# yunjinli/TRASE

Hardware: AMD Instinct MI355X
Metric: views/sec (fwd+bwd), 1080p, 300k Gaussians, 32-d feat (higher is better)
Workload: dtype f32 (channel contractions: 3-product bf16-split MFMA, fp32 accumulate)

## Files before the change

### include/trase_rast.h

```cpp
#ifndef TRASE_RAST_H
#define TRASE_RAST_H

#include <stddef.h>
#include <stdint.h>

#ifdef __cplusplus
extern "C" {
#endif

typedef void* trase_stream_t;

enum {
  TRASE_OK = 0,
  TRASE_ERR_INVALID = -1,
  TRASE_ERR_UNSUPPORTED = -2,
  TRASE_ERR_WORKSPACE = -3,
  TRASE_ERR_HIP = -4
};

typedef struct TraseRastSettings {
  int32_t image_height;
  int32_t image_width;
  float tanfovx;
  float tanfovy;
// ... 294 lines not shown
                               float* dL_dC_F, int32_t device, trase_stream_t stream);

int trase_nnfm_sizes(int32_t C, int32_t N1, int32_t N2, size_t* ws_bytes);
int trase_nnfm_forward(const float* feat1, const float* feats2, int32_t C, int32_t N1, int32_t N2, float* loss, void* ws,
                       size_t ws_bytes, int32_t device, trase_stream_t stream);
int trase_nnfm_backward(const float* feat1, const float* feats2, int32_t C, int32_t N1, int32_t N2, const float* g_loss,
                        const void* ws, size_t ws_bytes, float* dL_dfeat1, int32_t device, trase_stream_t stream);

int trase_adam_step(int32_t count, float* const* params, const float* const* grads, float* const* exp_avg,
                    float* const* exp_avg_sq, const int64_t* numel, const float* lr, const int64_t* step, double beta1,
                    double beta2, float eps, int32_t device, trase_stream_t stream);
int trase_adam_step_guarded(int32_t count, float* const* params, const float* const* grads, float* const* exp_avg,
                            float* const* exp_avg_sq, const int64_t* numel, const float* lr, const int64_t* step, double beta1,
                            double beta2, float eps, const void* guard, int32_t device, trase_stream_t stream);

int trase_prof_enable(int enable);
int trase_prof_report(char* buf, size_t buf_bytes);

int trase_selftest(int32_t device, trase_stream_t stream, char* msg, size_t msg_bytes);

int trase_selftest_sort(const uint32_t* keys, const uint32_t* vals, uint32_t n, uint32_t cap, int32_t bit_lo, int32_t bit_hi,
                        int32_t digit_bits, int32_t hist_copies, int32_t start, uint32_t flag_key, int32_t use_flag,
                        uint32_t sentinel, uint32_t* keys_out, uint32_t* vals_out, uint32_t* result, int32_t device,
                        trase_stream_t stream);
int trase_selftest_tile_ranges(const uint32_t* keys, uint32_t n, uint32_t cap, int32_t T, int32_t clear, uint32_t* ranges,
                               uint32_t* dbg, int32_t device, trase_stream_t stream);
int trase_selftest_zero_bytes(void* p, size_t bytes, int32_t device, trase_stream_t stream);

int trase_selftest_compact_live(const uint32_t* tiles, const uint32_t* keys, int32_t P, uint32_t* keys_out, uint32_t* ids_out,
                                uint32_t* live_ids_out, uint32_t* hdr_out, int32_t device, trase_stream_t stream);
int trase_selftest_scan_tiles(const uint32_t* tiles, const uint32_t* ids, const int32_t* radii, const float* xy, int32_t P,
                              uint32_t n_live, uint32_t cap, int32_t pack_bits, int32_t gx, int32_t gy, uint32_t overflow_in,
                              uint32_t* offsets_out, uint32_t* block_sums_out, uint32_t* hdr_out, int32_t device,
                              trase_stream_t stream);

const char* trase_last_error(void);
const char* trase_version(void);

int trase_densify_stats(const float* viewspace_grad, const int32_t* radii, float* xyz_gradient_accum, float* denom,
                        float* max_radii2D, int32_t P, int32_t device, trase_stream_t stream);
int trase_densify_stats_guarded(const float* viewspace_grad, const int32_t* radii, float* xyz_gradient_accum, float* denom,
                                float* max_radii2D, int32_t P, const void* guard, int32_t device, trase_stream_t stream);
int trase_densify_sizes(int32_t P, size_t* ws_bytes);
int trase_densify_plan(const float* xyz_gradient_accum, const float* denom, const float* scaling, const float* opacity,
                       int32_t P, float grad_threshold, float dense_extent, float min_opacity, int32_t use_screen_size,
                       float big_extent, int32_t* counts, void* ws, size_t ws_bytes, int32_t device,
                       trase_stream_t stream);
// ... 212 lines not shown
```

### trase_amd/_lib.py

```python
from __future__ import annotations

import ctypes as C
import os

import torch

_HERE = os.path.dirname(os.path.abspath(__file__))
LIB_PATH = os.environ.get("TRASE_RAST_LIB") or os.path.join(_HERE, "lib", "libtrase_rast.so")

c_float_p = C.POINTER(C.c_float)
FRAME_PLANAR = 1
LAYERS_MAX = 10
RIGID_STATE_FLOATS = 16


class RastSettings(C.Structure):
    _fields_ = [
        ("image_height", C.c_int32), ("image_width", C.c_int32),
        ("tanfovx", C.c_float), ("tanfovy", C.c_float),
        ("bg", C.c_void_p), ("scale_modifier", C.c_float),
        ("viewmatrix", C.c_void_p), ("projmatrix", C.c_void_p),
        ("sh_degree", C.c_int32), ("campos", C.c_void_p),
        ("prefiltered", C.c_int32), ("debug", C.c_int32),
        ("device", C.c_int32), ("variant", C.c_int32),
# ... 330 lines not shown
    ("trase_compose_sizes", C.c_int, [C.POINTER(C.c_int32), C.c_int32, C.c_int32, C.POINTER(C.c_int64)]),
    ("trase_compose_part", C.c_int, [C.POINTER(ComposePart), C.c_int64, C.c_int64, C.c_void_p, C.c_void_p, C.c_void_p, C.c_void_p,
                                     C.c_void_p, C.c_void_p, C.c_int32, C.c_void_p]),
    ("trase_evaluate_frame", C.c_int, [C.POINTER(EvalFrame), C.POINTER(RastWorkspace), C.c_int32, C.c_void_p]),
    ("trase_layers_pack", C.c_int, [C.POINTER(C.c_void_p), C.c_int32, C.c_int32, C.c_void_p, C.c_int32, C.c_void_p]),
    ("trase_layers_finish", C.c_int, [C.c_void_p, C.POINTER(RastWorkspace), C.c_void_p, C.c_int32, C.c_int32, C.c_int32, C.c_void_p,
                                      C.c_void_p, C.c_void_p, C.c_int32, C.c_void_p]),
    ("trase_fps_sample", C.c_int, [C.c_void_p, C.c_int32, C.c_void_p, C.c_int32, C.c_void_p, C.c_int32, C.c_void_p, C.c_void_p,
                                   C.c_void_p, C.c_int32, C.c_void_p]),
    ("trase_trajectory_append", C.c_int, [C.c_void_p, C.c_int32, C.c_void_p, C.c_int32, C.c_void_p, C.c_int32, C.c_void_p]),
    ("trase_trajectory_draw", C.c_int, [C.c_void_p, C.c_int32, C.c_int32, C.c_int32, C.c_int32, C.POINTER(C.c_double * 16),
                                        C.c_int32, C.c_int32, C.c_void_p, C.c_void_p, C.c_void_p, C.c_int32, C.c_void_p]),
    ("trase_present_frame", C.c_int, [C.c_void_p, C.c_int32, C.c_int32, C.c_int32, C.c_int32, C.c_int32, C.c_void_p, C.c_void_p,
                                      C.c_void_p, C.c_float, C.c_void_p, C.c_void_p, C.c_int32, C.c_void_p]),
    ("trase_adam_step", C.c_int, [C.c_int32, C.c_void_p, C.c_void_p, C.c_void_p, C.c_void_p, C.c_void_p, C.c_void_p,
                                  C.c_void_p, C.c_double, C.c_double, C.c_float, C.c_int32, C.c_void_p]),
    ("trase_adam_step_guarded", C.c_int, [C.c_int32, C.c_void_p, C.c_void_p, C.c_void_p, C.c_void_p, C.c_void_p, C.c_void_p,
                                          C.c_void_p, C.c_double, C.c_double, C.c_float, C.c_void_p, C.c_int32, C.c_void_p]),
    ("trase_prof_enable", C.c_int, [C.c_int]),
    ("trase_prof_report", C.c_int, [C.c_char_p, C.c_size_t]),
    ("trase_selftest", C.c_int, [C.c_int32, C.c_void_p, C.c_char_p, C.c_size_t]),
    ("trase_selftest_sort", C.c_int, [C.c_void_p, C.c_void_p, C.c_uint32, C.c_uint32, C.c_int32, C.c_int32, C.c_int32, C.c_int32,
                                      C.c_int32, C.c_uint32, C.c_int32, C.c_uint32, C.c_void_p, C.c_void_p,
                                      C.POINTER(C.c_uint32 * 3), C.c_int32, C.c_void_p]),
    ("trase_selftest_tile_ranges", C.c_int, [C.c_void_p, C.c_uint32, C.c_uint32, C.c_int32, C.c_int32, C.c_void_p,
                                             C.POINTER(C.c_uint32 * 3), C.c_int32, C.c_void_p]),
    ("trase_selftest_zero_bytes", C.c_int, [C.c_void_p, C.c_size_t, C.c_int32, C.c_void_p]),
    ("trase_selftest_compact_live", C.c_int, [C.c_void_p, C.c_void_p, C.c_int32, C.c_void_p, C.c_void_p, C.c_void_p,
                                              C.POINTER(C.c_uint32 * 5), C.c_int32, C.c_void_p]),
    ("trase_selftest_scan_tiles", C.c_int, [C.c_void_p, C.c_void_p, C.c_void_p, C.c_void_p, C.c_int32, C.c_uint32, C.c_uint32,
                                            C.c_int32, C.c_int32, C.c_int32, C.c_uint32, C.c_void_p, C.c_void_p,
                                            C.POINTER(C.c_uint32 * 5), C.c_int32, C.c_void_p]),
    ("trase_last_error", C.c_char_p, []),
    ("trase_version", C.c_char_p, []),
]

_lib = None


def load() -> C.CDLL:
    global _lib
    if _lib is not None:
        return _lib
    if not os.path.exists(LIB_PATH):
        raise RuntimeError(
            f"trase_amd: HIP library not built: {LIB_PATH} is missing. Run "
            "`python -c 'import __graft_entry__ as g; g.build()'` (or `make -C trase_amd/csrc`). "
# ... 27 lines not shown
```

### trase_amd/csrc/binning.hip

```cpp
#include <stdlib.h>

#include "common.h"

namespace trase {

constexpr int RS_WAVES = RS_THREADS / WAVE;
constexpr int RS_SEG = WAVE * RS_ITEMS;

__device__ __forceinline__ uint32_t dev_n(const uint32_t* n_ptr, uint32_t cap) {
  const uint32_t n = *n_ptr;
  return n < cap ? n : cap;
}

__device__ __forceinline__ uint32_t rs_tile(uint32_t b, uint32_t nb_live) {
#ifdef TRASE_RS_NO_XCD_MAP
  return b;
#else
  return (uint32_t)xcd_block((int)b, (int)nb_live);
#endif
}

template <int DB, bool SMALL = false>
__global__ __launch_bounds__(RS_THREADS) void radix_hist_kernel(const uint32_t* __restrict__ keys,
                                                                const uint32_t* __restrict__ n_ptr, uint32_t cap,
                                                                int shift, uint32_t mask, uint32_t* __restrict__ hist,
                                                                uint32_t* __restrict__ digit_total, int nb_max,
                                                                uint32_t flag_key = 0u, uint32_t* __restrict__ flag_word = nullptr,
                                                                uint32_t* __restrict__ zero_from = nullptr, uint32_t zero_words = 0u) {
  constexpr int ND = 1 << DB;
  for (uint32_t i = blockIdx.x * RS_THREADS + threadIdx.x; i < zero_words; i += gridDim.x * RS_THREADS) zero_from[i] = 0u;
  const uint32_t n = dev_n(n_ptr, cap);
  const uint32_t nb_live = (n + RS_TILE - 1) / RS_TILE;
  if (blockIdx.x >= nb_live) return;
  const uint32_t tile = SMALL ? blockIdx.x : rs_tile(blockIdx.x, nb_live);
  const uint32_t base = tile * RS_TILE;
  __shared__ uint32_t h[ND];
#pragma unroll
  for (int d = threadIdx.x; d < ND; d += RS_THREADS) h[d] = 0;
  __syncthreads();
  const unsigned lane = threadIdx.x & 63;
  uint32_t kk[RS_ITEMS];
#pragma unroll
  for (int i = 0; i < RS_ITEMS; ++i) {
    const uint32_t idx = base + i * RS_THREADS + threadIdx.x;
    kk[i] = idx < n ? keys[idx] : 0u;
  }
#pragma unroll
  for (int i = 0; i < RS_ITEMS; ++i) {
    const uint32_t idx = base + i * RS_THREADS + threadIdx.x;
    const bool valid = idx < n;
    if (flag_word && valid && kk[i] == flag_key) atomicOr(flag_word, 2u);
    const uint32_t dg = valid ? ((kk[i] >> shift) & mask) : 0xffffffffu;
    const uint32_t prev = (uint32_t)__shfl_up((int)dg, 1);
    const bool start = valid && (lane == 0 || prev != dg);
    const unsigned long long starts = __ballot(start);
    const unsigned long long vmask = __ballot(valid);
    if (start) {
      const unsigned long long later = (lane == 63) ? 0ull : (starts >> (lane + 1));
      const unsigned nvalid = (unsigned)__popcll(vmask);
      const unsigned next = later ? (lane + 1 + (unsigned)__builtin_ctzll(later)) : nvalid;
      atomicAdd(&h[dg], next - lane);
    }
  }
  __syncthreads();
#pragma unroll
  for (int d = threadIdx.x; d < ND; d += RS_THREADS) hist[(size_t)d * nb_max + tile] = h[d];
}

__device__ __forceinline__ uint32_t block256_incl_scan(uint32_t v, uint32_t* part ) {
  const int lane = threadIdx.x & 63, wave = threadIdx.x >> 6;
  uint32_t x = v;
#pragma unroll
  for (int o = 1; o < 64; o <<= 1) {
    const uint32_t y = (uint32_t)__shfl_up((int)x, o);
    if (lane >= o) x += y;
  }
  if (lane == 63) part[wave] = x;
  __syncthreads();
  uint32_t add = 0;
#pragma unroll
  for (int w = 0; w < 3; ++w) add += (w < wave) ? part[w] : 0u;
  __syncthreads();
  return x + add;
}

__global__ __launch_bounds__(256) void radix_scan_kernel(const uint32_t* __restrict__ n_ptr, uint32_t cap,
                                                         uint32_t* __restrict__ hist,
                                                         uint32_t* __restrict__ digit_total, int nb_max) {
  const uint32_t n = dev_n(n_ptr, cap);
// ... 13 lines not shown
#pragma unroll
    for (int u = 0; u < 32; ++u) v[u] = (b_lo + u < b_hi) ? row[b_lo + u] : 0u;
#pragma unroll
    for (int u = 0; u < 32; ++u) mine += v[u];
    incl = block256_incl_scan(mine, sh);
    run = incl - mine;
#pragma unroll
    for (int u = 0; u < 32; ++u) {
      if (b_lo + u < b_hi) row[b_lo + u] = run;
      run += v[u];
    }
  } else {
    for (int b = b_lo; b < b_hi; ++b) mine += row[b];
    incl = block256_incl_scan(mine, sh);
    run = incl - mine;
    for (int b = b_lo; b < b_hi; ++b) { const uint32_t v = row[b]; row[b] = run; run += v; }
  }
  if (threadIdx.x == 255) carry = incl;
  __syncthreads();
  if (threadIdx.x == 0) digit_total[d] = carry;
}

template <bool IOTA, int DB, bool SMALL = false>
__global__ __launch_bounds__(RS_THREADS) void radix_scatter_kernel(
    const uint32_t* __restrict__ keys_in, const uint32_t* __restrict__ vals_in, uint32_t* __restrict__ keys_out,
    uint32_t* __restrict__ vals_out, const uint32_t* __restrict__ n_ptr, uint32_t cap, int shift, uint32_t mask,
    const uint32_t* __restrict__ hist, const uint32_t* __restrict__ digit_total, int nb_max,
    uint32_t* __restrict__ hist_next = nullptr, int shift_next = 0, uint32_t mask_next = 0u) {
  constexpr int ND = 1 << DB;
  constexpr int DPT = ND / RS_THREADS;
  const uint32_t n = dev_n(n_ptr, cap);
  const uint32_t nb_live = (n + RS_TILE - 1) / RS_TILE;
  if (blockIdx.x >= nb_live) return;
  const uint32_t tile = SMALL ? blockIdx.x : rs_tile(blockIdx.x, nb_live);
  const uint32_t base = tile * RS_TILE;
  __shared__ uint32_t wcount[RS_WAVES][ND];
  const int wave = threadIdx.x >> 6;
  const unsigned lane = threadIdx.x & 63;
#pragma unroll
  for (int w = 0; w < RS_WAVES; ++w)
#pragma unroll
    for (int d = threadIdx.x; d < ND; d += RS_THREADS) wcount[w][d] = 0;
  __syncthreads();
  uint32_t k[RS_ITEMS], v[RS_ITEMS], rk[RS_ITEMS];
  const unsigned long long lt = lanemask_lt();
  volatile uint32_t* cnt = wcount[wave];
  uint32_t my_digit_total[DPT], my_hist[DPT];
  if constexpr (SMALL) {
    const int nb = (int)((n + RS_TILE - 1) / RS_TILE);
#pragma unroll
    for (int j = 0; j < DPT; ++j) {
      const uint32_t* row = hist + (size_t)(threadIdx.x * DPT + j) * nb_max;
      uint32_t before = 0, total = 0;
      for (int b0 = 0; b0 < nb; b0 += 8) {
        uint32_t v8[8];
#pragma unroll
        for (int u = 0; u < 8; ++u) v8[u] = (b0 + u < nb) ? row[b0 + u] : 0u;
#pragma unroll
        for (int u = 0; u < 8; ++u) { total += v8[u]; before += (b0 + u < (int)tile) ? v8[u] : 0u; }
      }
      my_digit_total[j] = total; my_hist[j] = before;
    }
  } else {
#pragma unroll
  for (int j = 0; j < DPT; ++j) {
    my_digit_total[j] = digit_total[threadIdx.x * DPT + j];
    my_hist[j] = hist[(size_t)(threadIdx.x * DPT + j) * nb_max + tile];
  }
  }
#pragma unroll
  for (int i = 0; i < RS_ITEMS; ++i) {
    const uint32_t idx = base + wave * RS_SEG + i * WAVE + lane;
    const bool valid = idx < n;
    k[i] = valid ? keys_in[idx] : 0xffffffffu;
    v[i] = valid ? (IOTA ? idx : vals_in[idx]) : 0u;
  }
#pragma unroll
  for (int i = 0; i < RS_ITEMS; ++i) {
    const uint32_t idx = base + wave * RS_SEG + i * WAVE + lane;
    const bool valid = idx < n;
    const uint32_t dg = (k[i] >> shift) & mask;
    unsigned long long peers = __ballot(valid);
    const uint32_t dg0 = __builtin_amdgcn_readfirstlane(dg);
    if (!__all(!valid || dg == dg0)) {
#pragma unroll
      for (int bit = 0; bit < DB; ++bit) {
        const bool set = (dg >> bit) & 1u;
        const unsigned long long bal = __ballot(set);
        peers &= set ? bal : ~bal;
      }
    }
    const uint32_t in_round = (uint32_t)__popcll(peers & lt);
    const uint32_t total = (uint32_t)__popcll(peers);
    uint32_t old = 0;
    if (valid) {
      old = cnt[dg];
      if (in_round == 0) cnt[dg] = old + total;
    }
    rk[i] = old + in_round;
    __builtin_amdgcn_wave_barrier();
  }
  __syncthreads();
  __shared__ uint32_t gbase[ND], lstart[ND];
  __shared__ uint32_t st_k[RS_TILE], st_v[RS_TILE];
  __shared__ uint32_t part_a[4], part_b[4];
  {
    uint32_t cnt_d[DPT], sum_l = 0, sum_g = 0;
#pragma unroll
    for (int j = 0; j < DPT; ++j) {
      const int d = threadIdx.x * DPT + j;
      uint32_t tot = 0;
#pragma unroll
      for (int w = 0; w < RS_WAVES; ++w) {
        const uint32_t c = wcount[w][d];
        wcount[w][d] = tot;
        tot += c;
      }
      cnt_d[j] = tot;
      sum_l += tot;
      sum_g += my_digit_total[j];
    }
    uint32_t run_l = block256_incl_scan(sum_l, part_a) - sum_l;
    uint32_t run_g = block256_incl_scan(sum_g, part_b) - sum_g;
#pragma unroll
    for (int j = 0; j < DPT; ++j) {
      const int d = threadIdx.x * DPT + j;
      lstart[d] = run_l;
      gbase[d] = run_g + my_hist[j];
      run_l += cnt_d[j];
      run_g += my_digit_total[j];
    }
  }
  __syncthreads();
#pragma unroll
  for (int i = 0; i < RS_ITEMS; ++i) {
    const uint32_t idx = base + wave * RS_SEG + i * WAVE + lane;
    if (idx < n) {
      const uint32_t dg = (k[i] >> shift) & mask;
      const uint32_t lp = lstart[dg] + wcount[wave][dg] + rk[i];
      st_k[lp] = k[i];
      st_v[lp] = v[i];
    }
  }
  __syncthreads();
  const uint32_t nblk = min((uint32_t)RS_TILE, n - base);
  for (uint32_t j = threadIdx.x; j < nblk; j += RS_THREADS) {
    const uint32_t kk = st_k[j];
    const uint32_t dg = (kk >> shift) & mask;
    const uint32_t dst = gbase[dg] + (j - lstart[dg]);
    keys_out[dst] = kk;
    vals_out[dst] = st_v[j];
    if constexpr (SMALL) {
      if (hist_next) {
        const uint32_t word = ((kk >> shift_next) & mask_next) * (uint32_t)nb_max + dst / RS_TILE;
        const uint32_t prev = (uint32_t)__shfl_up((int)word, 1);
        const bool start = lane == 0 || prev != word;
        const unsigned long long starts = __ballot(start), act = __ballot(true);
        if (start) {
          const unsigned long long later = (lane == 63) ? 0ull : (starts >> (lane + 1));
          const unsigned nact = (unsigned)__popcll(act);
          const unsigned next = later ? (lane + 1 + (unsigned)__builtin_ctzll(later)) : nact;
          atomicAdd(hist_next + word, next - lane);
        }
      }
    }
  }
}

__global__ __launch_bounds__(256) void zero_bytes_kernel(uint8_t* __restrict__ p, size_t bytes) {
  const size_t head = ((size_t)(-(intptr_t)p) & 15u) < bytes ? ((size_t)(-(intptr_t)p) & 15u) : bytes;
  const size_t n16 = (bytes - head) >> 4;
  uint4* q = reinterpret_cast<uint4*>(p + head);
// ... 18 lines not shown
  TRASE_POST_LAUNCH("fill_u32", stream, 0);
  return TRASE_OK;
}
__global__ __launch_bounds__(256) void split_pair_ids_kernel(const uint32_t* __restrict__ sorted, int P, uint32_t* __restrict__ ids0,
                                                             uint32_t* __restrict__ ids1) {
  const int i = blockIdx.x * 256 + threadIdx.x;
  if (i >= 2 * P) return;
  const uint32_t v = sorted[i];
  if (i < P) ids0[i] = v; else ids1[i - P] = v - (uint32_t)P;
}
int launch_split_pair_ids(const LaunchCtx& c, const uint32_t* sorted, int P, uint32_t* ids0, uint32_t* ids1) {
  TRASE_LAUNCH("split_pair_ids", c.stream, c.debug, split_pair_ids_kernel, dim3((2 * P + 255) / 256), dim3(256), 0, sorted, P, ids0, ids1);
  return TRASE_OK;
}

int radix_passes(int bit_lo, int bit_hi, int digit_bits) { return (bit_hi - bit_lo + digit_bits - 1) / digit_bits; }
bool radix_sort_is_short(int nb, int hist_copies, int passes) {
  static const bool small_off = [] { const char* e = getenv("TRASE_SORT_SMALL"); return e && atoi(e) == 0; }();
  return nb <= RS_SMALL_NB && hist_copies >= passes && !small_off;
}

template <int DB>
static int radix_sort_pairs_t(const LaunchCtx& c, const SortBufs& t, const uint32_t* n_ptr, uint32_t n_cap, int bit_lo, int bit_hi,
                              bool vals_are_iota, int start, int* out_idx, uint32_t flag_key, uint32_t* flag_word) {
  constexpr int ND = 1 << DB;
  int cur = start;
  const int nb = (int)((n_cap + RS_TILE - 1) / RS_TILE);
  if (nb > t.nb_max) { set_error("radix_sort_pairs: nb %d > nb_max %d", nb, t.nb_max); return TRASE_ERR_WORKSPACE; }
  const int passes = radix_passes(bit_lo, bit_hi, DB);
  if (passes > RS_MAX_PASSES) return TRASE_ERR_INVALID;
  if (radix_sort_is_short(nb, t.hist_copies, passes)) {
    const size_t hw = (size_t)ND * t.nb_max;
    for (int p = 0; p < passes; ++p) {
      const int shift = bit_lo + DB * p;
      const int nbits = (bit_hi - shift) < DB ? (bit_hi - shift) : DB;
      const uint32_t mask = (1u << nbits) - 1u;
      const int shift_n = shift + DB;
      const int nbits_n = (bit_hi - shift_n) < DB ? (bit_hi - shift_n) : DB;
      uint32_t* hist_p = t.hist + hw * p;
      uint32_t* hist_n = (p + 1 < passes) ? t.hist + hw * (p + 1) : nullptr;
      if (p == 0)
        TRASE_LAUNCH("radix_hist", c.stream, c.debug, (radix_hist_kernel<DB, true>), dim3(nb), dim3(RS_THREADS), 0, t.keys[cur], n_ptr, n_cap, shift, mask, hist_p,
                     t.digit_total, t.nb_max, flag_key, flag_word, t.hist + hw, (uint32_t)(hw * (passes - 1)));
      const uint32_t mask_n = hist_n ? ((1u << nbits_n) - 1u) : 0u;
      TRASE_LAUNCHES("radix_scatter", c.stream, c.debug,
        if (vals_are_iota && p == 0)
          hipLaunchKernelGGL((radix_scatter_kernel<true, DB, true>), dim3(nb), dim3(RS_THREADS), 0, c.stream, t.keys[cur], t.vals[cur],
                             t.keys[cur ^ 1], t.vals[cur ^ 1], n_ptr, n_cap, shift, mask, hist_p, t.digit_total, t.nb_max, hist_n, shift_n, mask_n);
        else
          hipLaunchKernelGGL((radix_scatter_kernel<false, DB, true>), dim3(nb), dim3(RS_THREADS), 0, c.stream, t.keys[cur], t.vals[cur],
                             t.keys[cur ^ 1], t.vals[cur ^ 1], n_ptr, n_cap, shift, mask, hist_p, t.digit_total, t.nb_max, hist_n, shift_n, mask_n));
      cur ^= 1;
    }
    *out_idx = cur;
    return TRASE_OK;
  }
  for (int p = 0; p < passes; ++p) {
    const int shift = bit_lo + DB * p;
    const int nbits = (bit_hi - shift) < DB ? (bit_hi - shift) : DB;
    const uint32_t mask = (1u << nbits) - 1u;
    uint32_t* dt = t.digit_total + ND * p;
    uint32_t* vout = t.vals[cur ^ 1];
    TRASE_LAUNCH("radix_hist", c.stream, c.debug, radix_hist_kernel<DB>, dim3(nb), dim3(RS_THREADS), 0, t.keys[cur], n_ptr, n_cap, shift,
                 mask, t.hist, dt, t.nb_max, flag_key, p == 0 ? flag_word : (uint32_t*)nullptr);
    TRASE_LAUNCH("radix_scan", c.stream, c.debug, radix_scan_kernel, dim3(ND), dim3(256), 0, n_ptr, n_cap, t.hist, dt, t.nb_max);
    TRASE_LAUNCHES("radix_scatter", c.stream, c.debug,
      if (vals_are_iota && p == 0)
        hipLaunchKernelGGL((radix_scatter_kernel<true, DB>), dim3(nb), dim3(RS_THREADS), 0, c.stream, t.keys[cur],
                           t.vals[cur], t.keys[cur ^ 1], vout, n_ptr, n_cap, shift, mask, t.hist, dt, t.nb_max);
      else
        hipLaunchKernelGGL((radix_scatter_kernel<false, DB>), dim3(nb), dim3(RS_THREADS), 0, c.stream, t.keys[cur],
                           t.vals[cur], t.keys[cur ^ 1], vout, n_ptr, n_cap, shift, mask, t.hist, dt, t.nb_max));
    cur ^= 1;
  }
  *out_idx = cur;
  return TRASE_OK;
}

int radix_sort_pairs(const LaunchCtx& c, const SortBufs& t, const uint32_t* n_ptr, uint32_t n_cap, int bit_lo, int bit_hi,
                     bool vals_are_iota, int* out_idx, int digit_bits, int start, uint32_t flag_key, uint32_t* flag_word) {
  if (digit_bits == 9) return radix_sort_pairs_t<9>(c, t, n_ptr, n_cap, bit_lo, bit_hi, vals_are_iota, start, out_idx, flag_key, flag_word);
  if (digit_bits == 8) return radix_sort_pairs_t<8>(c, t, n_ptr, n_cap, bit_lo, bit_hi, vals_are_iota, start, out_idx, flag_key, flag_word);
  set_error("radix_sort_pairs: digit_bits %d", digit_bits);
  return TRASE_ERR_INVALID;
}

constexpr int SC_THREADS = 256;
constexpr int SC_ITEMS = 4;
constexpr int SC_TILE = SC_THREADS * SC_ITEMS;

__global__ __launch_bounds__(SC_THREADS) void compact_count_kernel(const uint32_t* __restrict__ tiles, int P,
                                                                   uint32_t* __restrict__ block_cnt) {
  const int base = blockIdx.x * SC_TILE + threadIdx.x * SC_ITEMS;
  uint32_t c = 0;
  if (base + SC_ITEMS <= P) {
    const uint4 t = *reinterpret_cast<const uint4*>(tiles + base);
    c = (t.x != 0) + (t.y != 0) + (t.z != 0) + (t.w != 0);
  } else {
#pragma unroll
    for (int k = 0; k < SC_ITEMS; ++k) c += (base + k < P && tiles[base + k] != 0) ? 1u : 0u;
  }
#pragma unroll
  for (int o = 32; o > 0; o >>= 1) c += (uint32_t)__shfl_xor((int)c, o);
  __shared__ uint32_t part[SC_THREADS / 64];
  if ((threadIdx.x & 63) == 0) part[threadIdx.x >> 6] = c;
// ... 506 lines not shown
```

### trase_amd/csrc/common.h

```cpp
#pragma once

#include <hip/hip_runtime.h>
#include <stdint.h>
#include <stdio.h>

#include "../../include/trase_rast.h"
#include "gs_math.h"

namespace trase {

constexpr int WAVE = 64;

template <int CTRL, int ROW_MASK = 0xf>
__device__ __forceinline__ float dpp_f(float v) {
  return __builtin_bit_cast(float, __builtin_amdgcn_update_dpp(0, __builtin_bit_cast(int, v), CTRL, ROW_MASK, 0xf, false));
}

__device__ __forceinline__ float wave_sum_lane63(float v) {
  v += dpp_f<0x111>(v);
  v += dpp_f<0x112>(v);
  v += dpp_f<0x114>(v);
  v += dpp_f<0x118>(v);
  v += dpp_f<0x142, 0xa>(v);
  v += dpp_f<0x143, 0xc>(v);
// ... 258 lines not shown
  uint32_t* point_list;
  uint32_t* pair_slot;
  uint2* ranges;
  const uint32_t* id_end = nullptr;
};
struct ImgBuf {
  float* final_T;
  uint32_t* n_contrib;
};
struct SortBufs {
  uint32_t* keys[2];
  uint32_t* vals[2];
  uint32_t* hist;
  uint32_t* digit_total;
  int nb_max;
  int hist_copies;
};
#ifndef TRASE_RS_ITEMS
#define TRASE_RS_ITEMS 8
#endif
constexpr int RS_THREADS = 256, RS_ITEMS = TRASE_RS_ITEMS;
constexpr int RS_TILE = RS_THREADS * RS_ITEMS;
constexpr int RS_MAX_PASSES = 8;
inline int rs_blocks(size_t n) { return (int)((n + RS_TILE - 1) / RS_TILE); }
constexpr int RS_SMALL_NB = 16;
constexpr int RS_SMALL_COPIES = 4;
inline int rs_hist_copies(int nb) { return nb <= RS_SMALL_NB ? RS_SMALL_COPIES : 1; }
enum { SORT_KEYS = 1, SORT_VALS = 2, SORT_HIST = 4, SORT_ALL = 7 };
inline void sort_layout(WsCursor& w, SortBufs& s, size_t n, int parts = SORT_ALL, int digit_bits = 8, int hist_copies = 0) {
  if (parts & SORT_KEYS) for (int i = 0; i < 2; ++i) s.keys[i] = w.take<uint32_t>(n);
  if (parts & SORT_VALS) for (int i = 0; i < 2; ++i) s.vals[i] = w.take<uint32_t>(n);
  if (!(parts & SORT_HIST)) return;
  const size_t digits = (size_t)1 << digit_bits;
  s.nb_max = rs_blocks(n);
  s.hist_copies = hist_copies ? hist_copies : rs_hist_copies(s.nb_max);
  s.hist = w.take<uint32_t>(digits * s.nb_max * s.hist_copies);
  s.digit_total = w.take<uint32_t>(digits * RS_MAX_PASSES);
}
struct PreBuf {
  SortBufs sort;
  uint32_t* offsets;
  uint32_t* id_end;
  uint32_t* block_sums;
  uint32_t* block_R;
  uint32_t* block_max;
  uint32_t* live_ids;
// ... 38 lines not shown
  asm("v_cvt_pk_bf16_f32 %0, %1, %2" : "=v"(lo) : "v"(ra), "v"(rb));
}
__device__ __forceinline__ float4 split_rgbd(float r, float g, float b, float d) {
  unsigned h01, l01, h23, l23;
  split_pk(r, g, h01, l01);
  split_pk(b, d, h23, l23);
  return make_float4(__uint_as_float(h01), __uint_as_float(h23), __uint_as_float(l01), __uint_as_float(l23));
}
int launch_feature_table(const LaunchCtx& c, const float* feats, const uint32_t* tiles, int P, uint32_t* ftab);

int launch_preprocess_fwd(const LaunchCtx& c, const TraseRastSettings& s, const TraseRastInputs& in, int32_t* radii,
                          const GeomBuf& g, uint32_t* depth_keys, bool key27);
int launch_preprocess_bwd(const LaunchCtx& c, const TraseRastSettings& s, const TraseRastInputs& in, const int32_t* radii,
                          const GeomBuf& g, const float* acc, const TraseRastGrads& gr);


int launch_preprocess_bwd_raw(const LaunchCtx& c, const TraseRastSettings& s, const TraseRastRawInputs& raw,
                              const int32_t* radii, const GeomBuf& g, const float* acc, const TraseRastRawGrads& gr,
                              int p_begin = 0, int p_end = -1, int zero_dead_feats = 0, const uint32_t* live_ids = nullptr);
int launch_zero_live_rows(const LaunchCtx& c, const GeomBuf& g, const PreBuf& pre, int P, int F, const TraseRastRawGrads& gr);

int radix_sort_pairs(const LaunchCtx& c, const SortBufs& t, const uint32_t* n_ptr, uint32_t n_cap, int bit_lo, int bit_hi,
                     bool vals_are_iota, int* out_idx, int digit_bits = 8, int start = 0, uint32_t flag_key = 0u,
                     uint32_t* flag_word = nullptr);
int launch_zero_bytes(void* p, size_t bytes, hipStream_t stream);
int launch_fill_u32(uint32_t* p, uint32_t v, hipStream_t stream);
constexpr int LABEL_SUMS_MAX = 128;
struct LabelSumsWs { float* slabs; float* total; int32_t* slot; };
size_t label_sums_layout(void* ws, int N, int D, int S, LabelSumsWs& w);
int launch_label_sums(const float* X, int N, int D, const int32_t* ids, const int32_t* sel, int S, const LabelSumsWs& w, hipStream_t stream);
int launch_evaluate(const TraseEvalFrame& f, const float* final_T, hipStream_t stream);
constexpr int LAYERS_F = 32;
int launch_layers_pack(const float* const* tables, int L, int P, float* out, hipStream_t stream);
int launch_layers_finish(float* planes, const float* final_T, const float* bg, int L, int W, int H, const float* image,
                         uint8_t* image_u8, uint8_t* layers_u8, hipStream_t stream);
int launch_split_pair_ids(const LaunchCtx& c, const uint32_t* sorted, int P, uint32_t* ids0, uint32_t* ids1);
int radix_passes(int bit_lo, int bit_hi, int digit_bits = 8);
bool radix_sort_is_short(int nb, int hist_copies, int passes);
struct DepthSortCfg { int key_bits, digit_bits, passes, start; };
inline DepthSortCfg depth_sort_cfg(int variant) {
  return (variant & TRASE_VARIANT_DEPTH32) ? DepthSortCfg{32, 8, 4, 0} : DepthSortCfg{27, 9, 3, 1};
}
constexpr int DEPTH_MAX_DIGIT_BITS = 9;
constexpr uint32_t DEPTH27_BASE = 0x3e4ccccdu, DEPTH27_SAT = 0x07fffffeu, DEPTH27_DEAD = 0x07ffffffu;
__host__ __device__ inline uint32_t depth_sort_key(float z, bool key27) {
  const uint32_t bits = __builtin_bit_cast(uint32_t, z);
  if (!key27) return bits;
// ... 34 lines not shown
```

### trase_amd/csrc/selftest.hip

```cpp
#include <string>

#include "common.h"

namespace trase {

__global__ void selftest_wave_kernel(float* outf, unsigned long long* outu) {
  const unsigned lane = threadIdx.x;
  const float v = (float)(lane + 1);
  const float s63 = wave_sum_lane63(v);
  if (lane == 63) outf[0] = s63;
  const float all = wave_sum_all(v);
  if (lane == 0) outf[1] = all;
  const unsigned long long bal = __ballot(lane & 1u);
  if (lane == 0) outu[0] = bal;
  float pc = (float)__popcll(lanemask_lt());
  pc = wave_sum_all(pc);
  if (lane == 0) outf[2] = pc;
  float li = wave_sum_all((float)lane_id());
  if (lane == 0) outf[3] = li;
  const float sa = wave_scan_add(v);
  float bad = (sa == 0.5f * (float)((lane + 1) * (lane + 2))) ? 0.f : 1.f;
  const float sm = wave_scan_mul((lane & 1u) ? 1.0f : 1.03125f);
  float want = 1.0f;
  for (unsigned k = 0; k <= lane; k += 2) want *= 1.03125f;
// ... 70 lines not shown
  int mfma_bad = 0;
  for (int i = 0; i < 32; ++i)
    for (int j = 0; j < 32; ++j) {
      const float want = (float)i * (float)(j + 1) + ((float)i + 100.f) * ((float)(j + 1) * 0.5f);
      if (hm[i * 32 + j] != want) ++mfma_bad;
    }
  expect("mfma 32x32x2 f32 layout mismatches", mfma_bad, 0.0);
  if (msg && msg_bytes) {
    snprintf(msg, msg_bytes, "%s", report.c_str());
  }
  return bad;
}

namespace {
struct DevBlock {
  void* p = nullptr;
  ~DevBlock() { if (p) hipFree(p); }
};
}

extern "C" int trase_selftest_sort(const uint32_t* keys, const uint32_t* vals, uint32_t n, uint32_t cap, int32_t bit_lo,
                                   int32_t bit_hi, int32_t digit_bits, int32_t hist_copies, int32_t start, uint32_t flag_key,
                                   int32_t use_flag, uint32_t sentinel, uint32_t* keys_out, uint32_t* vals_out, uint32_t* result,
                                   int32_t device, trase_stream_t stream_) {
  hipStream_t stream = (hipStream_t)stream_;
  if (!keys || !keys_out || !vals_out || !result || cap < 1 || (digit_bits != 8 && digit_bits != 9) || bit_lo < 0 ||
      bit_hi <= bit_lo || bit_hi > 32 || hist_copies < 0 || (start != 0 && start != 1)) {
    set_error("trase_selftest_sort: bad arguments");
    return TRASE_ERR_INVALID;
  }
  TRASE_CHECK(hipSetDevice(device));
  SortBufs s{};
  uint32_t *n_dev = nullptr, *flag_dev = nullptr;
  auto layout = [&](void* ws) {
    WsCursor w(ws);
    sort_layout(w, s, cap, SORT_ALL, digit_bits, hist_copies);
    n_dev = w.take<uint32_t>(1);
    flag_dev = w.take<uint32_t>(1);
    return w.bytes();
  };
  const size_t bytes = layout(nullptr);
  DevBlock blk;
  TRASE_CHECK(hipMalloc(&blk.p, bytes));
  layout(blk.p);
  TRASE_CHECK(hipMemsetAsync(blk.p, 0xCD, bytes, stream));
  const size_t cb = sizeof(uint32_t) * (size_t)cap;
  TRASE_CHECK(hipMemsetD32Async((hipDeviceptr_t)s.keys[start ^ 1], (int)sentinel, cap, stream));
  TRASE_CHECK(hipMemsetD32Async((hipDeviceptr_t)s.vals[start ^ 1], (int)sentinel, cap, stream));
  TRASE_CHECK(hipMemcpyAsync(s.keys[start], keys, cb, hipMemcpyDeviceToDevice, stream));
  if (vals) TRASE_CHECK(hipMemcpyAsync(s.vals[start], vals, cb, hipMemcpyDeviceToDevice, stream));
  else TRASE_CHECK(hipMemsetD32Async((hipDeviceptr_t)s.vals[start], (int)sentinel, cap, stream));
  TRASE_CHECK(hipMemcpyAsync(n_dev, &n, sizeof(n), hipMemcpyHostToDevice, stream));
  TRASE_CHECK(hipMemsetAsync(flag_dev, 0, sizeof(uint32_t), stream));
  const LaunchCtx c{stream, 0, 0};
  int out_idx = -1;
  const int rc = radix_sort_pairs(c, s, n_dev, cap, bit_lo, bit_hi, vals == nullptr, &out_idx, digit_bits, start, flag_key,
                                  use_flag ? flag_dev : nullptr);
  if (rc != TRASE_OK) { hipStreamSynchronize(stream); return rc; }
  uint32_t flag = 0;
  TRASE_CHECK(hipMemcpyAsync(keys_out, s.keys[out_idx], cb, hipMemcpyDeviceToDevice, stream));
  TRASE_CHECK(hipMemcpyAsync(vals_out, s.vals[out_idx], cb, hipMemcpyDeviceToDevice, stream));
  TRASE_CHECK(hipMemcpyAsync(&flag, flag_dev, sizeof(flag), hipMemcpyDeviceToHost, stream));
  TRASE_CHECK(hipStreamSynchronize(stream));
  result[0] = (uint32_t)out_idx;
  result[1] = flag;
  result[2] = radix_sort_is_short(rs_blocks(cap), s.hist_copies, radix_passes(bit_lo, bit_hi, digit_bits)) ? 1u : 0u;
  return TRASE_OK;
}

extern "C" int trase_selftest_tile_ranges(const uint32_t* keys, uint32_t n, uint32_t cap, int32_t T, int32_t clear,
                                          uint32_t* ranges, uint32_t* dbg, int32_t device, trase_stream_t stream_) {
  hipStream_t stream = (hipStream_t)stream_;
  if (!keys || !ranges || !dbg || T < 1) {
    set_error("trase_selftest_tile_ranges: bad arguments");
    return TRASE_ERR_INVALID;
  }
  TRASE_CHECK(hipSetDevice(device));
  DevBlock blk;
  TRASE_CHECK(hipMalloc(&blk.p, 4 * sizeof(uint32_t)));
  uint32_t* w = (uint32_t*)blk.p;
// ... 98 lines not shown
```

### trase_amd/rasterizer.py

```python
from __future__ import annotations

import ctypes as C
import os
from typing import NamedTuple, Optional

import torch
import torch.nn as nn

from . import _lib


class GaussianRasterizationSettings(NamedTuple):
    image_height: int
    image_width: int
    tanfovx: float
    tanfovy: float
    bg: torch.Tensor
    scale_modifier: float
    viewmatrix: torch.Tensor
    projmatrix: torch.Tensor
    sh_degree: int
    campos: torch.Tensor
    prefiltered: bool
    debug: bool
# ... 609 lines not shown


def profile_enable(mode: int):
    _lib.check(_lib.load().trase_prof_enable(int(mode)), "trase_prof_enable")


def profile_report() -> dict:
    import json
    buf = C.create_string_buffer(1 << 16)
    _lib.check(_lib.load().trase_prof_report(buf, len(buf)), "trase_prof_report")
    return json.loads(buf.value.decode())


def selftest(device=None) -> str:
    dev = torch.cuda.current_device() if device is None else device
    buf = C.create_string_buffer(4096)
    rc = _lib.load().trase_selftest(dev, _stream(torch.device("cuda", dev)), buf, len(buf))
    msg = buf.value.decode()
    if rc != 0:
        raise RuntimeError(f"trase_selftest failed ({rc}):\n{msg}\n{_lib.last_error()}")
    return msg


def selftest_sort(keys, vals, n, bit_lo, bit_hi, digit_bits=8, hist_copies=0, start=0, flag_key=None, sentinel=0xDEADBEEF):
    assert keys.is_cuda and keys.dtype == torch.int32 and keys.is_contiguous()
    assert vals is None or (vals.is_cuda and vals.dtype == torch.int32 and vals.is_contiguous() and vals.shape == keys.shape)
    dev = keys.device
    d = dev.index if dev.index is not None else torch.cuda.current_device()
    keys_out, vals_out = torch.empty_like(keys), torch.empty_like(keys)
    res = (C.c_uint32 * 3)()
    _lib.check(_lib.load().trase_selftest_sort(
        _lib.ptr(keys), _lib.ptr(vals), int(n), keys.numel(), int(bit_lo), int(bit_hi), int(digit_bits), int(hist_copies),
        int(start), 0 if flag_key is None else int(flag_key), 0 if flag_key is None else 1, int(sentinel), _lib.ptr(keys_out),
        _lib.ptr(vals_out), C.byref(res), d, _stream(dev)), "trase_selftest_sort")
    return keys_out, vals_out, int(res[0]), int(res[1]), bool(res[2])


def selftest_tile_ranges(keys, n, cap, ranges, T, clear=True):
    assert keys.is_cuda and keys.dtype == torch.int32 and keys.is_contiguous()
    assert ranges.is_cuda and ranges.dtype == torch.int32 and ranges.is_contiguous() and ranges.numel() >= 2 * T
    dev = keys.device
    d = dev.index if dev.index is not None else torch.cuda.current_device()
    dbg = (C.c_uint32 * 3)()
    _lib.check(_lib.load().trase_selftest_tile_ranges(_lib.ptr(keys), int(n), int(cap), int(T), int(bool(clear)), _lib.ptr(ranges),
                                                      C.byref(dbg), d, _stream(dev)), "trase_selftest_tile_ranges")
    return [int(x) for x in dbg]


def selftest_zero_bytes(buf, offset, nbytes):
    assert buf.is_cuda and buf.dtype == torch.uint8 and buf.is_contiguous() and 0 <= offset and offset + nbytes <= buf.numel()
    dev = buf.device
    d = dev.index if dev.index is not None else torch.cuda.current_device()
    _lib.check(_lib.load().trase_selftest_zero_bytes(C.c_void_p(buf.data_ptr() + offset), int(nbytes), d, _stream(dev)),
               "trase_selftest_zero_bytes")


def _hdr5(res) -> dict:
# ... 66 lines not shown
```

Baseline: 952.1.

## Make radix histogram persistent with prefetch and add LDS match ranking in scatter

The radix histogram kernel becomes grid-strided over tiles with a capped grid (default 2048). It prefetches the next tile's keys into registers while the current tile is counted, and resets the shared histogram between tiles. The scatter kernel aliases its per-wave count tables onto the key/value staging buffer to cut LDS footprint. For 8-bit non-small passes it ranks digit peers with LDS atomic-or bitmasks, adds a higher launch-bounds occupancy hint, and folds the local start into gbase to simplify the output address. Risks are extra register pressure from the prefetch and LDS atomic contention in the new ranking.

Result: no change. 954.1 (median of 6 runs) (+0.2%).

```diff
diff --git a/include/trase_rast.h b/include/trase_rast.h
--- a/include/trase_rast.h
+++ b/include/trase_rast.h
@@ -340,7 +340,7 @@
 int trase_selftest_sort(const uint32_t* keys, const uint32_t* vals, uint32_t n, uint32_t cap, int32_t bit_lo, int32_t bit_hi,
                         int32_t digit_bits, int32_t hist_copies, int32_t start, uint32_t flag_key, int32_t use_flag,
                         uint32_t sentinel, uint32_t* keys_out, uint32_t* vals_out, uint32_t* result, int32_t device,
-                        trase_stream_t stream);
+                        trase_stream_t stream, int32_t hist_grid);
 int trase_selftest_tile_ranges(const uint32_t* keys, uint32_t n, uint32_t cap, int32_t T, int32_t clear, uint32_t* ranges,
                                uint32_t* dbg, int32_t device, trase_stream_t stream);
 int trase_selftest_zero_bytes(void* p, size_t bytes, int32_t device, trase_stream_t stream);
diff --git a/trase_amd/_lib.py b/trase_amd/_lib.py
--- a/trase_amd/_lib.py
+++ b/trase_amd/_lib.py
@@ -376,7 +376,7 @@
     ("trase_selftest", C.c_int, [C.c_int32, C.c_void_p, C.c_char_p, C.c_size_t]),
     ("trase_selftest_sort", C.c_int, [C.c_void_p, C.c_void_p, C.c_uint32, C.c_uint32, C.c_int32, C.c_int32, C.c_int32, C.c_int32,
                                       C.c_int32, C.c_uint32, C.c_int32, C.c_uint32, C.c_void_p, C.c_void_p,
-                                      C.POINTER(C.c_uint32 * 3), C.c_int32, C.c_void_p]),
+                                      C.POINTER(C.c_uint32 * 3), C.c_int32, C.c_void_p, C.c_int32]),
     ("trase_selftest_tile_ranges", C.c_int, [C.c_void_p, C.c_uint32, C.c_uint32, C.c_int32, C.c_int32, C.c_void_p,
                                              C.POINTER(C.c_uint32 * 3), C.c_int32, C.c_void_p]),
     ("trase_selftest_zero_bytes", C.c_int, [C.c_void_p, C.c_size_t, C.c_int32, C.c_void_p]),
diff --git a/trase_amd/csrc/binning.hip b/trase_amd/csrc/binning.hip
--- a/trase_amd/csrc/binning.hip
+++ b/trase_amd/csrc/binning.hip
@@ -32,39 +32,59 @@
   const uint32_t n = dev_n(n_ptr, cap);
   const uint32_t nb_live = (n + RS_TILE - 1) / RS_TILE;
   if (blockIdx.x >= nb_live) return;
-  const uint32_t tile = SMALL ? blockIdx.x : rs_tile(blockIdx.x, nb_live);
-  const uint32_t base = tile * RS_TILE;
   __shared__ uint32_t h[ND];
 #pragma unroll
   for (int d = threadIdx.x; d < ND; d += RS_THREADS) h[d] = 0;
-  __syncthreads();
   const unsigned lane = threadIdx.x & 63;
-  uint32_t kk[RS_ITEMS];
+  uint32_t kk[RS_ITEMS], kn[RS_ITEMS];
+  uint32_t v = blockIdx.x;
+  uint32_t tile = SMALL ? v : rs_tile(v, nb_live);
 #pragma unroll
   for (int i = 0; i < RS_ITEMS; ++i) {
-    const uint32_t idx = base + i * RS_THREADS + threadIdx.x;
+    const uint32_t idx = tile * RS_TILE + i * RS_THREADS + threadIdx.x;
     kk[i] = idx < n ? keys[idx] : 0u;
   }
-#pragma unroll
-  for (int i = 0; i < RS_ITEMS; ++i) {
-    const uint32_t idx = base + i * RS_THREADS + threadIdx.x;
-    const bool valid = idx < n;
-    if (flag_word && valid && kk[i] == flag_key) atomicOr(flag_word, 2u);
-    const uint32_t dg = valid ? ((kk[i] >> shift) & mask) : 0xffffffffu;
-    const uint32_t prev = (uint32_t)__shfl_up((int)dg, 1);
-    const bool start = valid && (lane == 0 || prev != dg);
-    const unsigned long long starts = __ballot(start);
-    const unsigned long long vmask = __ballot(valid);
-    if (start) {
-      const unsigned long long later = (lane == 63) ? 0ull : (starts >> (lane + 1));
-      const unsigned nvalid = (unsigned)__popcll(vmask);
-      const unsigned next = later ? (lane + 1 + (unsigned)__builtin_ctzll(later)) : nvalid;
-      atomicAdd(&h[dg], next - lane);
-    }
-  }
-  __syncthreads();
-#pragma unroll
-  for (int d = threadIdx.x; d < ND; d += RS_THREADS) hist[(size_t)d * nb_max + tile] = h[d];
+  for (;;) {
+    const uint32_t base = tile * RS_TILE;
+    const uint32_t v_next = v + gridDim.x;
+    const bool more = v_next < nb_live;
+    const uint32_t tile_next = more ? (SMALL ? v_next : rs_tile(v_next, nb_live)) : 0u;
+    if (more) {
+#pragma unroll
+      for (int i = 0; i < RS_ITEMS; ++i) {
+        const uint32_t idx = tile_next * RS_TILE + i * RS_THREADS + threadIdx.x;
+        kn[i] = idx < n ? keys[idx] : 0u;
+      }
+    }
+    __syncthreads();
+#pragma unroll
+    for (int i = 0; i < RS_ITEMS; ++i) {
+      const uint32_t idx = base + i * RS_THREADS + threadIdx.x;
+      const bool valid = idx < n;
+      if (flag_word && valid && kk[i] == flag_key) atomicOr(flag_word, 2u);
+      const uint32_t dg = valid ? ((kk[i] >> shift) & mask) : 0xffffffffu;
+      const uint32_t prev = (uint32_t)__shfl_up((int)dg, 1);
+      const bool start = valid && (lane == 0 || prev != dg);
+      const unsigned long long starts = __ballot(start);
+      const unsigned long long vmask = __ballot(valid);
+      if (start) {
+        const unsigned long long later = (lane == 63) ? 0ull : (starts >> (lane + 1));
+        const unsigned nvalid = (unsigned)__popcll(vmask);
+        const unsigned next = later ? (lane + 1 + (unsigned)__builtin_ctzll(later)) : nvalid;
+        atomicAdd(&h[dg], next - lane);
+      }
+    }
+    __syncthreads();
+    for (int d = threadIdx.x; d < ND; d += RS_THREADS) {
+      hist[(size_t)d * nb_max + tile] = h[d];
+      h[d] = 0;
+    }
+    if (!more) break;
+#pragma unroll
+    for (int i = 0; i < RS_ITEMS; ++i) kk[i] = kn[i];
+    v = v_next;
+    tile = tile_next;
+  }
 }
 
 __device__ __forceinline__ uint32_t block256_incl_scan(uint32_t v, uint32_t* part ) {
@@ -124,7 +144,7 @@
 }
 
 template <bool IOTA, int DB, bool SMALL = false>
-__global__ __launch_bounds__(RS_THREADS) void radix_scatter_kernel(
+__global__ __launch_bounds__(RS_THREADS, DB == 8 && !SMALL ? 8 : 1) void radix_scatter_kernel(
     const uint32_t* __restrict__ keys_in, const uint32_t* __restrict__ vals_in, uint32_t* __restrict__ keys_out,
     uint32_t* __restrict__ vals_out, const uint32_t* __restrict__ n_ptr, uint32_t cap, int shift, uint32_t mask,
     const uint32_t* __restrict__ hist, const uint32_t* __restrict__ digit_total, int nb_max,
@@ -136,13 +156,17 @@
   if (blockIdx.x >= nb_live) return;
   const uint32_t tile = SMALL ? blockIdx.x : rs_tile(blockIdx.x, nb_live);
   const uint32_t base = tile * RS_TILE;
-  __shared__ uint32_t wcount[RS_WAVES][ND];
+  __shared__ uint32_t stage[2 * RS_TILE];
+  uint32_t (*wcount)[ND] = reinterpret_cast<uint32_t (*)[ND]>(stage);
+  uint32_t* const st_k = stage;
+  uint32_t* const st_v = stage + RS_TILE;
   const int wave = threadIdx.x >> 6;
   const unsigned lane = threadIdx.x & 63;
-#pragma unroll
-  for (int w = 0; w < RS_WAVES; ++w)
-#pragma unroll
-    for (int d = threadIdx.x; d < ND; d += RS_THREADS) wcount[w][d] = 0;
+  constexpr bool LDS_MATCH = DB == 8 && !SMALL;
+  constexpr int CLEAR_WORDS = RS_WAVES * ND * (LDS_MATCH ? 3 : 1);
+  static_assert(CLEAR_WORDS <= 2 * RS_TILE, "the ranking's tables live in the staging buffer");
+#pragma unroll
+  for (int d = threadIdx.x; d < CLEAR_WORDS; d += RS_THREADS) stage[d] = 0;
   __syncthreads();
   uint32_t k[RS_ITEMS], v[RS_ITEMS], rk[RS_ITEMS];
   const unsigned long long lt = lanemask_lt();
@@ -177,6 +201,31 @@
     k[i] = valid ? keys_in[idx] : 0xffffffffu;
     v[i] = valid ? (IOTA ? idx : vals_in[idx]) : 0u;
   }
+  if constexpr (LDS_MATCH) {
+    unsigned long long* wbits = reinterpret_cast<unsigned long long*>(stage + RS_WAVES * ND) + wave * ND;
+    volatile unsigned long long* vbits = wbits;
+    const unsigned long long me = 1ull << lane;
+#pragma unroll
+    for (int i = 0; i < RS_ITEMS; ++i) {
+      const uint32_t idx = base + wave * RS_SEG + i * WAVE + lane;
+      const bool valid = idx < n;
+      const uint32_t dg = (k[i] >> shift) & mask;
+      if (valid) __hip_atomic_fetch_or(&wbits[dg], me, __ATOMIC_RELAXED, __HIP_MEMORY_SCOPE_WORKGROUP);
+      __builtin_amdgcn_wave_barrier();
+      const unsigned long long peers = valid ? vbits[dg] : 0ull;
+      const uint32_t in_round = (uint32_t)__popcll(peers & lt);
+      uint32_t old = 0;
+      if (valid) {
+        old = cnt[dg];
+        if (in_round == 0) {
+          cnt[dg] = old + (uint32_t)__popcll(peers);
+          vbits[dg] = 0ull;
+        }
+      }
+      rk[i] = old + in_round;
+      __builtin_amdgcn_wave_barrier();
+    }
+  } else {
 #pragma unroll
   for (int i = 0; i < RS_ITEMS; ++i) {
     const uint32_t idx = base + wave * RS_SEG + i * WAVE + lane;
@@ -202,9 +251,9 @@
     rk[i] = old + in_round;
     __builtin_amdgcn_wave_barrier();
   }
+  }
   __syncthreads();
   __shared__ uint32_t gbase[ND], lstart[ND];
-  __shared__ uint32_t st_k[RS_TILE], st_v[RS_TILE];
   __shared__ uint32_t part_a[4], part_b[4];
   {
     uint32_t cnt_d[DPT], sum_l = 0, sum_g = 0;
@@ -228,7 +277,7 @@
     for (int j = 0; j < DPT; ++j) {
       const int d = threadIdx.x * DPT + j;
       lstart[d] = run_l;
-      gbase[d] = run_g + my_hist[j];
+      gbase[d] = run_g + my_hist[j] - run_l;
       run_l += cnt_d[j];
       run_g += my_digit_total[j];
     }
@@ -239,9 +288,16 @@
     const uint32_t idx = base + wave * RS_SEG + i * WAVE + lane;
     if (idx < n) {
       const uint32_t dg = (k[i] >> shift) & mask;
-      const uint32_t lp = lstart[dg] + wcount[wave][dg] + rk[i];
-      st_k[lp] = k[i];
-      st_v[lp] = v[i];
+      rk[i] += lstart[dg] + wcount[wave][dg];
+    }
+  }
+  __syncthreads();
+#pragma unroll
+  for (int i = 0; i < RS_ITEMS; ++i) {
+    const uint32_t idx = base + wave * RS_SEG + i * WAVE + lane;
+    if (idx < n) {
+      st_k[rk[i]] = k[i];
+      st_v[rk[i]] = v[i];
     }
   }
   __syncthreads();
@@ -249,7 +305,7 @@
   for (uint32_t j = threadIdx.x; j < nblk; j += RS_THREADS) {
     const uint32_t kk = st_k[j];
     const uint32_t dg = (kk >> shift) & mask;
-    const uint32_t dst = gbase[dg] + (j - lstart[dg]);
+    const uint32_t dst = gbase[dg] + j;
     keys_out[dst] = kk;
     vals_out[dst] = st_v[j];
     if constexpr (SMALL) {
@@ -314,10 +370,11 @@
 
 template <int DB>
 static int radix_sort_pairs_t(const LaunchCtx& c, const SortBufs& t, const uint32_t* n_ptr, uint32_t n_cap, int bit_lo, int bit_hi,
-                              bool vals_are_iota, int start, int* out_idx, uint32_t flag_key, uint32_t* flag_word) {
+                              bool vals_are_iota, int start, int* out_idx, uint32_t flag_key, uint32_t* flag_word, int hist_grid) {
   constexpr int ND = 1 << DB;
   int cur = start;
   const int nb = (int)((n_cap + RS_TILE - 1) / RS_TILE);
+  const int nb_hist = nb < hist_grid ? nb : hist_grid;
   if (nb > t.nb_max) { set_error("radix_sort_pairs: nb %d > nb_max %d", nb, t.nb_max); return TRASE_ERR_WORKSPACE; }
   const int passes = radix_passes(bit_lo, bit_hi, DB);
   if (passes > RS_MAX_PASSES) return TRASE_ERR_INVALID;
@@ -332,7 +389,7 @@
       uint32_t* hist_p = t.hist + hw * p;
       uint32_t* hist_n = (p + 1 < passes) ? t.hist + hw * (p + 1) : nullptr;
       if (p == 0)
-        TRASE_LAUNCH("radix_hist", c.stream, c.debug, (radix_hist_kernel<DB, true>), dim3(nb), dim3(RS_THREADS), 0, t.keys[cur], n_ptr, n_cap, shift, mask, hist_p,
+        TRASE_LAUNCH("radix_hist", c.stream, c.debug, (radix_hist_kernel<DB, true>), dim3(nb_hist), dim3(RS_THREADS), 0, t.keys[cur], n_ptr, n_cap, shift, mask, hist_p,
                      t.digit_total, t.nb_max, flag_key, flag_word, t.hist + hw, (uint32_t)(hw * (passes - 1)));
       const uint32_t mask_n = hist_n ? ((1u << nbits_n) - 1u) : 0u;
       TRASE_LAUNCHES("radix_scatter", c.stream, c.debug,
@@ -353,7 +410,7 @@
     const uint32_t mask = (1u << nbits) - 1u;
     uint32_t* dt = t.digit_total + ND * p;
     uint32_t* vout = t.vals[cur ^ 1];
-    TRASE_LAUNCH("radix_hist", c.stream, c.debug, radix_hist_kernel<DB>, dim3(nb), dim3(RS_THREADS), 0, t.keys[cur], n_ptr, n_cap, shift,
+    TRASE_LAUNCH("radix_hist", c.stream, c.debug, radix_hist_kernel<DB>, dim3(nb_hist), dim3(RS_THREADS), 0, t.keys[cur], n_ptr, n_cap, shift,
                  mask, t.hist, dt, t.nb_max, flag_key, p == 0 ? flag_word : (uint32_t*)nullptr);
     TRASE_LAUNCH("radix_scan", c.stream, c.debug, radix_scan_kernel, dim3(ND), dim3(256), 0, n_ptr, n_cap, t.hist, dt, t.nb_max);
     TRASE_LAUNCHES("radix_scatter", c.stream, c.debug,
@@ -370,9 +427,11 @@
 }
 
 int radix_sort_pairs(const LaunchCtx& c, const SortBufs& t, const uint32_t* n_ptr, uint32_t n_cap, int bit_lo, int bit_hi,
-                     bool vals_are_iota, int* out_idx, int digit_bits, int start, uint32_t flag_key, uint32_t* flag_word) {
-  if (digit_bits == 9) return radix_sort_pairs_t<9>(c, t, n_ptr, n_cap, bit_lo, bit_hi, vals_are_iota, start, out_idx, flag_key, flag_word);
-  if (digit_bits == 8) return radix_sort_pairs_t<8>(c, t, n_ptr, n_cap, bit_lo, bit_hi, vals_are_iota, start, out_idx, flag_key, flag_word);
+                     bool vals_are_iota, int* out_idx, int digit_bits, int start, uint32_t flag_key, uint32_t* flag_word, int hist_grid) {
+  if (hist_grid < 0) { set_error("radix_sort_pairs: hist_grid %d", hist_grid); return TRASE_ERR_INVALID; }
+  if (hist_grid == 0) hist_grid = RS_HIST_GRID;
+  if (digit_bits == 9) return radix_sort_pairs_t<9>(c, t, n_ptr, n_cap, bit_lo, bit_hi, vals_are_iota, start, out_idx, flag_key, flag_word, hist_grid);
+  if (digit_bits == 8) return radix_sort_pairs_t<8>(c, t, n_ptr, n_cap, bit_lo, bit_hi, vals_are_iota, start, out_idx, flag_key, flag_word, hist_grid);
   set_error("radix_sort_pairs: digit_bits %d", digit_bits);
   return TRASE_ERR_INVALID;
 }
diff --git a/trase_amd/csrc/common.h b/trase_amd/csrc/common.h
--- a/trase_amd/csrc/common.h
+++ b/trase_amd/csrc/common.h
@@ -304,6 +304,7 @@
 constexpr int RS_THREADS = 256, RS_ITEMS = TRASE_RS_ITEMS;
 constexpr int RS_TILE = RS_THREADS * RS_ITEMS;
 constexpr int RS_MAX_PASSES = 8;
+constexpr int RS_HIST_GRID = 2048;
 inline int rs_blocks(size_t n) { return (int)((n + RS_TILE - 1) / RS_TILE); }
 constexpr int RS_SMALL_NB = 16;
 constexpr int RS_SMALL_COPIES = 4;
@@ -388,7 +389,8 @@
 
 int radix_sort_pairs(const LaunchCtx& c, const SortBufs& t, const uint32_t* n_ptr, uint32_t n_cap, int bit_lo, int bit_hi,
                      bool vals_are_iota, int* out_idx, int digit_bits = 8, int start = 0, uint32_t flag_key = 0u,
-                     uint32_t* flag_word = nullptr);
+                     uint32_t* flag_word = nullptr,
+                     int hist_grid = 0);
 int launch_zero_bytes(void* p, size_t bytes, hipStream_t stream);
 int launch_fill_u32(uint32_t* p, uint32_t v, hipStream_t stream);
 constexpr int LABEL_SUMS_MAX = 128;
diff --git a/trase_amd/csrc/selftest.hip b/trase_amd/csrc/selftest.hip
--- a/trase_amd/csrc/selftest.hip
+++ b/trase_amd/csrc/selftest.hip
@@ -116,10 +116,10 @@
 extern "C" int trase_selftest_sort(const uint32_t* keys, const uint32_t* vals, uint32_t n, uint32_t cap, int32_t bit_lo,
                                    int32_t bit_hi, int32_t digit_bits, int32_t hist_copies, int32_t start, uint32_t flag_key,
                                    int32_t use_flag, uint32_t sentinel, uint32_t* keys_out, uint32_t* vals_out, uint32_t* result,
-                                   int32_t device, trase_stream_t stream_) {
+                                   int32_t device, trase_stream_t stream_, int32_t hist_grid) {
   hipStream_t stream = (hipStream_t)stream_;
   if (!keys || !keys_out || !vals_out || !result || cap < 1 || (digit_bits != 8 && digit_bits != 9) || bit_lo < 0 ||
-      bit_hi <= bit_lo || bit_hi > 32 || hist_copies < 0 || (start != 0 && start != 1)) {
+      bit_hi <= bit_lo || bit_hi > 32 || hist_copies < 0 || (start != 0 && start != 1) || hist_grid < 0) {
     set_error("trase_selftest_sort: bad arguments");
     return TRASE_ERR_INVALID;
   }
@@ -149,7 +149,7 @@
   const LaunchCtx c{stream, 0, 0};
   int out_idx = -1;
   const int rc = radix_sort_pairs(c, s, n_dev, cap, bit_lo, bit_hi, vals == nullptr, &out_idx, digit_bits, start, flag_key,
-                                  use_flag ? flag_dev : nullptr);
+                                  use_flag ? flag_dev : nullptr, hist_grid);
   if (rc != TRASE_OK) { hipStreamSynchronize(stream); return rc; }
   uint32_t flag = 0;
   TRASE_CHECK(hipMemcpyAsync(keys_out, s.keys[out_idx], cb, hipMemcpyDeviceToDevice, stream));
diff --git a/trase_amd/rasterizer.py b/trase_amd/rasterizer.py
--- a/trase_amd/rasterizer.py
+++ b/trase_amd/rasterizer.py
@@ -655,7 +655,8 @@
     return msg
 
 
-def selftest_sort(keys, vals, n, bit_lo, bit_hi, digit_bits=8, hist_copies=0, start=0, flag_key=None, sentinel=0xDEADBEEF):
+def selftest_sort(keys, vals, n, bit_lo, bit_hi, digit_bits=8, hist_copies=0, start=0, flag_key=None, sentinel=0xDEADBEEF,
+                  hist_grid=0):
     assert keys.is_cuda and keys.dtype == torch.int32 and keys.is_contiguous()
     assert vals is None or (vals.is_cuda and vals.dtype == torch.int32 and vals.is_contiguous() and vals.shape == keys.shape)
     dev = keys.device
@@ -665,7 +666,7 @@
     _lib.check(_lib.load().trase_selftest_sort(
         _lib.ptr(keys), _lib.ptr(vals), int(n), keys.numel(), int(bit_lo), int(bit_hi), int(digit_bits), int(hist_copies),
         int(start), 0 if flag_key is None else int(flag_key), 0 if flag_key is None else 1, int(sentinel), _lib.ptr(keys_out),
-        _lib.ptr(vals_out), C.byref(res), d, _stream(dev)), "trase_selftest_sort")
+        _lib.ptr(vals_out), C.byref(res), d, _stream(dev), int(hist_grid)), "trase_selftest_sort")
     return keys_out, vals_out, int(res[0]), int(res[1]), bool(res[2])
 
 
```
